# levayz/ProtoSAM

Measured on AMD Instinct MI355X. Metric: query-slices/sec (512x512) end-to-end ProtoSAM infer, higher is better.
Workload: dtype f16

## Files before the change

### include/protosam_hip.h

```cpp
#ifndef PROTOSAM_HIP_H
#define PROTOSAM_HIP_H
#include <stddef.h>
#ifdef __cplusplus
extern "C" {
#endif

int psam_gemm_f16(const void* A, const void* W, const float* bias, void* out, const float* resid, const float* gamma,
                  int M, int N, int K, int lda, int ldw, int ldo, int ldr, int resid_mod, int out_seg,
                  int out_seg_stride, int out_seg_off, int epilogue, void* stream);
int psam_gemm_f16_heads(const void* A, const void* W, const float* bias, void* out, int M, int N, int K, int lda, int ldw,
                        int hd, void* stream);
int psam_gemm_f16_ln(const void* A, const void* W, const float* bias, void* out, const float* resid, const float* gamma,
                     int M, int N, int K, int lda, int ldw, int ldo, int ldr, int resid_mod, int out_seg,
                     int out_seg_stride, int out_seg_off, int epilogue, void* out16, int ld16, float* stats,
                     const float* ln_mr, const float* ln_s, void* stream);
int psam_ln_finalize(const float* stats, int M, int D, float eps, float* mr, void* stream);


int psam_gemm_splitk_ranges(int M, int N, int K);
int psam_gemm_f16_splitk_ln(const void* A, const void* W, const float* bias, float* x, int M, int N, int K, int lda, int ldw, int ldx,
                            int ks, float* ws, const float* ln_w, const float* ln_b, float eps, void* out16, int ld16, void* stream);

int psam_gemm_set_tile(int tile);
int psam_gemm_last_tile(int* tile);
// ... 23 lines not shown
#define PSAM_ATTN_KERNEL_STAGE64 0x200
#define PSAM_ATTN_KERNEL_QT4 0x400
#define PSAM_ATTN_KERNEL_V2 0x800
int psam_attention_last_kernel(int* id);
int psam_attention_fused_relpos(int B, int N, int H, int hd, int gh, int gw);

int psam_relpos(const void* qkv, const void* Rpack, float* rel_h, float* rel_w, void* relq, int B, int N, int H, int hd,
                int gw, int K, int windowed, float scale, int head_major, void* stream);

int psam_alp_bank(const float* sup, int ld, int h, int w, int C, const float* mask, const float* bmask, int MH, int MW,
                  int pool_w, int kernel_size, float thresh, float eps, float* bank, int cap, int* meta, int* slot_bg,
                  int* slot_fg, float* mres, int force_mode, void* stream);

int psam_alp_sim(const float* qry, long long q_bstride, int ld, int B, int npix, int C, const float* bank, int cap,
                 const int* meta, float eps, float sim_scale, float* part, float* pred, int which_only, void* stream);
int psam_alp_sim_pairs(const float* qry, long long q_bstride, int ld, int npix, int C, const void* tab, int n_entries,
                       int max_groups, float eps, float sim_scale, float* part, float* pred, void* stream);

int psam_patchify_bilinear(const float* img, int B, int C, int H, int W, int S, int P, int Kpad, void* out, void* stream);
int psam_bilinear_nchw(const float* in, int planes, int IH, int IW, int OH, int OW, float* out, void* stream);
int psam_resize2d(const float* in, int planes, int IH, int IW, int OH, int OW, int mode, float* out, void* stream);
int psam_bilinear_tokens(const float* in, long long in_bstride, int ld, int B, int ih, int iw, int C, int oh, int ow,
                         float* out, void* stream);
int psam_prob_argmax(const float* logits, int B, int IH, int IW, int OH, int OW, float* prob, void* pred, int* fg_sum,
                     void* stream);
int psam_broadcast_rows(const float* row, int D, float* out, int B, long long stride, long long off, void* stream);
int psam_prob2_argmax(const float* scores, int P, int IH, int IW, int OH, int OW, void* pred, float* pfg2, int* fg_sum,
                      float* prob, void* stream);
int psam_scores_prob_argmax(const float* scores, int P, int GH, int GW, int IH, int IW, int OH, int OW, float* prob, void* pred,
                            int* fg_sum, void* stream);
int psam_minmax(const float* x, int B, long long n_per_img, void* mm, void* stream);
int psam_sam_patchify(const float* img, const void* mm, int B, int S, int P, const float* mean3, const float* std3,
                      int quantise, void* out, void* u8out, void* stream);
int psam_normalize_chw(const void* x, int in_u8, int B, long long plane, const float* mean3, const float* std3,
                       float* y, void* stream);
int psam_im2col3x3(const void* in, int B, int H, int W, int C, void* out, void* stream);
int psam_cast_f16(const float* x, void* y, long long n, void* stream);
int psam_cast_f32(const void* x, float* y, long long n, void* stream);
int psam_gelu_f32(float* x, long long n, void* stream);
int psam_split_f16(const float* x, void* hi, void* lo, long long n, int write_hi, void* stream);

int psam_ccl(const void* pred, const float* pfg, int H, int W, int cap, int* labels, int* parent, int* counters,
             int* roots, int* acc_i, void* acc_u, double* acc_d, const int* fg_sum, double* tab, void* stream);
int psam_ccl_batch(const void* pred, const float* pfg, long long pfg_stride, int B, int H, int W, int cap, int* labels, int* parent,
                   int* counters, int* roots, int* acc_i, void* acc_u, double* acc_d, const int* fg_sum, double* tab, void* stream);

int psam_small_linear(const float* x, const float* x2, const float* W, const float* b, const float* resid, float* y,
                      int G, int M, int N, int K, long long xg, long long wg, long long bg, long long yg, int ldx,
                      int ldy, int act, void* stream);
int psam_small_linear_splitk(const float* x, const float* W, const float* b, const float* resid, float* y, float* parts, int M, int N,
                             int K, int ks, int ldx, int ldy, void* stream);
int psam_small_attention(const void* q, const float* k, const float* v, void* out, int B, int Tq, int Tk, int NH, int hd,
                         int ldq, int ldk, int ldv, int ldo, int q_f16, void* stream);
#define PSAM_MAX_PROMPT_TOKENS 256
int psam_token_attention(const void* q, const float* k, const float* v, void* out, int B, int Tq, int Tk, int NH, int hd,
                         int ldq, int ldk, int ldv, int ldo, int q_f16, void* stream);
int psam_t2i_attention(const float* q, const void* K, const void* V, float* out, int B, int T, int Nk, int NH,
                       int kv_f32, void* stream);
int psam_t2i_attention_split(const float* q, const void* K, const void* V, float* out, int B, int T, int Nk, int NH,
                             int kv_f32, int S, float* part, void* stream);
int psam_gemm_f32(const float* a, const float* a2, int a2_mod, const float* w, const float* bias, const float* resid,
                  float* out, int M, int N, int K, int lda, int ldw, int ldo, void* stream);
int psam_gemm_f32_heads(const float* a, const float* a2, int a2_mod, const float* w, const float* bias, float* out, int M, int N, int K,
                        int lda, int ldw, int nk, int hd, void* stream);

int psam_gemm_f32x3(const float* a, const float* a2, int a2_mod, const void* wh, const void* wl, const float* bias, const float* resid,
// ... 67 lines not shown
```

### protosam_amd/_lib.py

```python
import ctypes
import os

import torch

_HERE = os.path.dirname(os.path.abspath(__file__))
LIB_PATH = os.environ.get("PSAM_LIB_PATH") or os.path.join(_HERE, "libprotosam_hip.so")

c_void_p, c_int, c_float, c_longlong, c_size_t = ctypes.c_void_p, ctypes.c_int, ctypes.c_float, ctypes.c_longlong, ctypes.c_size_t

SIGNATURES = {
    "psam_gemm_f16": [c_void_p, c_void_p, c_void_p, c_void_p, c_void_p, c_void_p] + [c_int] * 12 + [c_void_p],
    "psam_gemm_f16_heads": [c_void_p, c_void_p, c_void_p, c_void_p] + [c_int] * 6 + [c_void_p],
    "psam_gemm_f16_ln": [c_void_p] * 6 + [c_int] * 12 + [c_void_p, c_int, c_void_p, c_void_p, c_void_p, c_void_p],
    "psam_ln_finalize": [c_void_p, c_int, c_int, c_float, c_void_p, c_void_p],
    "psam_gemm_splitk_ranges": [c_int, c_int, c_int],
    "psam_gemm_f16_splitk_ln": [c_void_p, c_void_p, c_void_p, c_void_p] + [c_int] * 7 + [c_void_p, c_void_p, c_void_p, c_float, c_void_p, c_int,
                                c_void_p],
    "psam_gemm_set_tile": [c_int],
    "psam_gemm_last_tile": [ctypes.POINTER(c_int)],
    "psam_gemm_asm_variant": [c_int],
    "psam_gemm_set_option": [ctypes.c_char_p, c_int],
    "psam_gemm_set_workspace": [c_void_p, c_size_t],
    "psam_layernorm": [c_void_p, c_void_p, c_void_p, c_void_p, c_void_p, c_int, c_int, c_int, c_int, c_float,
                       c_int, c_int, c_void_p],
# ... 44 lines not shown
                        c_void_p, c_void_p],
    "psam_im2col": [c_void_p] + [c_int] * 10 + [c_void_p, c_void_p],
    "psam_im2col_stem": [c_void_p, c_int, c_int, c_int, c_int, c_void_p, c_void_p],
    "psam_maxpool3x3s2": [c_void_p, c_int, c_int, c_int, c_int, c_void_p, c_void_p],
    "psam_rotate_nearest": [c_void_p, c_void_p, c_void_p, c_void_p, c_void_p, c_int, c_int, c_int, c_int, c_int, c_int,
                            c_int, c_void_p],
    "psam_resize_aa": [c_void_p, c_void_p, c_void_p, c_int, c_int, c_int, c_int, c_int, c_void_p],
    "psam_image_intake": [c_void_p, c_longlong, ctypes.POINTER(c_longlong), c_void_p, c_int, c_int, c_int, c_int, c_int,
                          ctypes.POINTER(c_float), ctypes.POINTER(c_float), c_void_p, c_void_p],
    "psam_volume_stats": [c_void_p, c_int, ctypes.c_longlong, c_float, c_float, c_void_p, c_void_p],
    "psam_volume_slices": [c_void_p, c_int, c_int, c_int, c_int, c_float, c_float, c_float, c_float, c_int, c_int, c_int,
                           c_void_p, c_void_p],
    "psam_neg_points": [c_void_p, c_void_p, c_void_p, c_int, c_int, c_int, c_int, c_float, c_void_p, c_void_p],
    "psam_neg_points_batch": [c_void_p, c_void_p, c_longlong, c_void_p] + [c_int] * 6 + [c_float, c_void_p, c_void_p],
    "psam_topk_points_workspace": [c_int, c_int, c_int, ctypes.POINTER(c_longlong)],
    "psam_topk_points_batch": [c_void_p, c_void_p, c_longlong, c_void_p] + [c_int] * 7 + [c_void_p, c_void_p, c_longlong, c_void_p],
    "psam_topk_points": [c_void_p, c_void_p, c_void_p] + [c_int] * 6 + [c_void_p, c_void_p, c_longlong, c_void_p],
    "psam_mask_downscale": [c_void_p, c_void_p, c_int, c_int, c_float, c_void_p, c_void_p],
    "psam_plane_stats": [c_void_p, c_int, c_int, c_int, c_float, c_float, c_void_p, c_void_p, c_void_p],
    "psam_rle_workspace": [c_int, c_int, ctypes.POINTER(c_longlong)],
    "psam_rle_count": [c_void_p, c_int, c_int, c_int, c_void_p, c_void_p, c_void_p],
    "psam_rle_write": [c_void_p, c_int, c_int, c_int, c_void_p, c_void_p, c_void_p, c_void_p],
    "psam_rle_decode": [c_void_p, c_void_p, c_int, c_int, c_int, c_void_p, c_void_p],
    "psam_seg_counts": [c_void_p, c_int, c_int, c_longlong, c_void_p, c_int, c_int, c_longlong, c_int, c_int, c_void_p, c_int,
                        c_void_p, c_void_p],
    "psam_mask_binarize": [c_void_p, c_void_p, c_int, c_int, c_int, c_int, c_int, c_int, c_float, c_void_p, c_void_p,
                           c_void_p, c_void_p],
    "psam_normalize_chw": [c_void_p, c_int, c_int, c_longlong, ctypes.POINTER(c_float), ctypes.POINTER(c_float),
                           c_void_p, c_void_p],
    "psam_ccl": [c_void_p, c_void_p, c_int, c_int, c_int] + [c_void_p] * 9 + [c_void_p],
    "psam_ccl_batch": [c_void_p, c_void_p, c_longlong, c_int, c_int, c_int, c_int] + [c_void_p] * 9 + [c_void_p],
    "psam_sam_patchify": [c_void_p, c_void_p, c_int, c_int, c_int, ctypes.POINTER(c_float), ctypes.POINTER(c_float),
                          c_int, c_void_p, c_void_p, c_void_p],
}

_lib = None


class HipExtensionMissing(RuntimeError):
    pass


def _preload_torch_hip_runtime():
    tl = os.path.join(os.path.dirname(torch.__file__), "lib", "libamdhip64.so")
    if os.path.exists(tl):
        ctypes.CDLL(tl, mode=ctypes.RTLD_GLOBAL)


def lib():
    global _lib
    if _lib is not None:
        return _lib
    if not os.path.exists(LIB_PATH):
        raise HipExtensionMissing(
            f"{LIB_PATH} not found: build it with `make -C protosam_amd/csrc` (or __graft_entry__.build()). "
            "protosam_amd has no CPU fallback.")
    _preload_torch_hip_runtime()
    L = ctypes.CDLL(LIB_PATH)
    for name, argtypes in SIGNATURES.items():
        fn = getattr(L, name)
        fn.argtypes = argtypes
        fn.restype = c_int
    _lib = L
    return L


# ... 4 lines not shown
```

### protosam_amd/csrc/resample.hip

```cpp
#include "common.h"
#include "interp.h"

__global__ void patchify_bilinear_kernel(const float* __restrict__ img, int B, int C, int H, int W, int S, int P,
                                         int Kpad, half_t* __restrict__ out) {
  const int npw = S / P;
  const int patch = blockIdx.x, b = blockIdx.y;
  const int py = patch / npw, px = patch % npw;
  const float sh = (float)H / (float)S, sw = (float)W / (float)S;
  half_t* o = out + ((size_t)b * npw * npw + patch) * Kpad;
  const int K = C * P * P;
  const bool same = (H == S && W == S);
  for (int k = threadIdx.x; k < Kpad; k += blockDim.x) {
    float v = 0.f;
    if (k < K) {
      int c = k / (P * P), r = k % (P * P);
      int y = py * P + r / P, x = px * P + r % P;
      const float* pl = img + ((size_t)b * C + c) * H * W;
      if (same) {
        v = pl[(size_t)y * W + x];
      } else {
        Lin ly = lin_src(y, sh, H), lx = lin_src(x, sw, W);
        v = bilerp(pl, W, ly, lx);
      }
    }
// ... 158 lines not shown
}
__global__ __launch_bounds__(256) void minmax_kernel(const float* __restrict__ x, size_t n_per_img,
                                                     uint32_t* __restrict__ mm) {
  const int b = blockIdx.y;
  const float* p = x + (size_t)b * n_per_img;
  float lo = INFINITY, hi = -INFINITY;
  const size_t n4 = ((reinterpret_cast<uintptr_t>(p) & 15) == 0) ? n_per_img / 4 : 0;
  for (size_t i = (size_t)blockIdx.x * blockDim.x + threadIdx.x; i < n4; i += (size_t)gridDim.x * blockDim.x) {
    const float4 v = reinterpret_cast<const float4*>(p)[i];
    lo = fminf(fminf(lo, v.x), fminf(fminf(v.y, v.z), v.w));
    hi = fmaxf(fmaxf(hi, v.x), fmaxf(fmaxf(v.y, v.z), v.w));
  }
  for (size_t i = n4 * 4 + (size_t)blockIdx.x * blockDim.x + threadIdx.x; i < n_per_img; i += (size_t)gridDim.x * blockDim.x) {
    float v = p[i];
    lo = fminf(lo, v);
    hi = fmaxf(hi, v);
  }
  lo = wave_min(lo);
  hi = wave_max(hi);
  __shared__ float red[2][4];
  if ((threadIdx.x & 63) == 0) {
    red[0][threadIdx.x >> 6] = lo;
    red[1][threadIdx.x >> 6] = hi;
  }
  __syncthreads();
  if (threadIdx.x == 0) {
    lo = fminf(fminf(red[0][0], red[0][1]), fminf(red[0][2], red[0][3]));
    hi = fmaxf(fmaxf(red[1][0], red[1][1]), fmaxf(red[1][2], red[1][3]));
    atomicMin(&mm[2 * b], f2ord(lo));
    atomicMax(&mm[2 * b + 1], f2ord(hi));
  }
}

__global__ void sam_patchify_kernel(const float* __restrict__ img, const uint32_t* __restrict__ mm, int S, int P,
                                    float m0, float m1, float m2, float s0, float s1, float s2, int quantise,
                                    half_t* __restrict__ out, uint8_t* __restrict__ u8out) {
  const int npw = S / P;
  const int patch = blockIdx.x, b = blockIdx.y;
  const int py = patch / npw, px = patch % npw;
  const float lo = ord2f(mm[2 * b]), hi = ord2f(mm[2 * b + 1]);
  const float rng = hi - lo;
  const int K = 3 * P * P;
  half_t* o = out + ((size_t)b * npw * npw + patch) * K;
  for (int k = threadIdx.x; k < K; k += blockDim.x) {
    int c = k / (P * P), r = k % (P * P);
    int y = py * P + r / P, x = px * P + r % P;
    float v = img[(((size_t)b * 3 + c) * S + y) * S + x];
    float q = (v - lo) / rng;
    if (quantise) {
      q = q * 255.0f;
      q = (float)(int)q;
      if (u8out) u8out[(((size_t)b * 3 + c) * S + y) * S + x] = (uint8_t)q;
    }
    const float mean = c == 0 ? m0 : (c == 1 ? m1 : m2);
    const float sd = c == 0 ? s0 : (c == 1 ? s1 : s2);
    o[k] = (half_t)((q - mean) / sd);
  }
}

extern "C" int psam_minmax(const float* x, int B, long long n_per_img, void* mm, void* stream) {
  if (B <= 0 || n_per_img <= 0) return PSAM_ERR_ARG;
  hipStream_t s = (hipStream_t)stream;
  hipLaunchKernelGGL(minmax_init_kernel, dim3((B + 63) / 64), dim3(64), 0, s, (uint32_t*)mm, B);
  int nb = (int)((n_per_img + 256 * 16 - 1) / (256 * 16));
  if (nb > 128) nb = 128;
  hipLaunchKernelGGL(minmax_kernel, dim3(nb, B), dim3(256), 0, s, x, (size_t)n_per_img, (uint32_t*)mm);
  return psam_launch_status();
}

extern "C" int psam_sam_patchify(const float* img, const void* mm, int B, int S, int P, const float* mean3,
                                 const float* std3, int quantise, void* out, void* u8out, void* stream) {
  if (B <= 0 || S <= 0 || P <= 0 || S % P || !mean3 || !std3) return PSAM_ERR_ARG;
  const int np = (S / P) * (S / P);
  hipLaunchKernelGGL(sam_patchify_kernel, dim3(np, B), dim3(256), 0, (hipStream_t)stream, img, (const uint32_t*)mm, S,
                     P, mean3[0], mean3[1], mean3[2], std3[0], std3[1], std3[2], quantise, (half_t*)out,
                     (uint8_t*)u8out);
  return psam_launch_status();
}

__global__ void im2col3x3_kernel(const half_t* __restrict__ in, int H, int W, int C, half_t* __restrict__ out) {
  const int pix = blockIdx.x, b = blockIdx.y;
  const int y = pix / W, x = pix % W;
  const int cv = C / 8;
  uint4* o = reinterpret_cast<uint4*>(out + ((size_t)b * H * W + pix) * 9 * C);
  for (int i = threadIdx.x; i < 9 * cv; i += blockDim.x) {
    int tap = i / cv, c = i % cv;
    int yy = y + tap / 3 - 1, xx = x + tap % 3 - 1;
    uint4 v = make_uint4(0, 0, 0, 0);
    if (yy >= 0 && yy < H && xx >= 0 && xx < W)
      v = reinterpret_cast<const uint4*>(in + ((size_t)b * H * W + (size_t)yy * W + xx) * C)[c];
    o[i] = v;
  }
}
extern "C" int psam_im2col3x3(const void* in, int B, int H, int W, int C, void* out, void* stream) {
  if (B <= 0 || H <= 0 || W <= 0 || C <= 0 || (C % 8) != 0) return PSAM_ERR_ARG;
  hipLaunchKernelGGL(im2col3x3_kernel, dim3(H * W, B), dim3(256), 0, (hipStream_t)stream, (const half_t*)in, H, W, C,
                     (half_t*)out);
  return psam_launch_status();
}

__global__ void cast_f16_kernel(const float* __restrict__ x, half_t* __restrict__ y, size_t n8) {
  size_t i = (size_t)blockIdx.x * blockDim.x + threadIdx.x;
  if (i >= n8) return;
  const float4 a = reinterpret_cast<const float4*>(x)[2 * i], b = reinterpret_cast<const float4*>(x)[2 * i + 1];
  half8_t h = {(half_t)a.x, (half_t)a.y, (half_t)a.z, (half_t)a.w, (half_t)b.x, (half_t)b.y, (half_t)b.z, (half_t)b.w};
  reinterpret_cast<half8_t*>(y)[i] = h;
}
extern "C" int psam_cast_f16(const float* x, void* y, long long n, void* stream) {
// ... 303 lines not shown
```

### protosam_amd/ops.py

```python
import torch

from . import _lib

EPI_F16, EPI_GELU_F16, EPI_F32, EPI_RELU_F16 = 0, 1, 2, 3


_raw_stream = getattr(torch._C, "_cuda_getCurrentRawStream", None)
_raw_device = getattr(torch._C, "_cuda_getDevice", None)


def _stream():
    if _raw_stream is not None and _raw_device is not None:
        return _raw_stream(_raw_device())
    return torch.cuda.current_stream().cuda_stream


class KernelTimer:

    def __init__(self):
        self.records = []
        self.tags = {}

    def start(self):
        e = torch.cuda.Event(enable_timing=True)
# ... 630 lines not shown
    st = _lib.lib().psam_prob2_argmax(_ptr(scores), P, scores.shape[2], scores.shape[3], OH, OW, _ptr(pred), _ptr(pfg2),
                                      _ptr(fg_sum), _ptr(prob), _stream())
    _tstop(h, P * (2 * scores.shape[2] * scores.shape[3] * 4 + OH * OW * (5 + (8 if prob is not None else 0))))
    _lib.check(st, "psam_prob2_argmax")
    return pred, pfg2


def scores_prob_argmax(scores, IH, IW, OH, OW, prob=None, pred=None, fg_sum=None):
    _req(scores, torch.float32, "scores")
    assert scores.is_contiguous() and scores.dim() == 4 and scores.shape[1] == 2
    P, dev = scores.shape[0], scores.device
    if prob is None:
        prob = torch.empty((P, 2, OH, OW), dtype=torch.float32, device=dev)
    if pred is None:
        pred = torch.empty((P, OH, OW), dtype=torch.uint8, device=dev)
    _req(prob, torch.float32, "prob")
    assert prob.is_contiguous() and prob.numel() >= P * 2 * OH * OW
    assert pred.dtype == torch.uint8 and pred.is_cuda and pred.is_contiguous() and pred.numel() >= P * OH * OW
    assert fg_sum is None or (fg_sum.dtype == torch.int32 and fg_sum.is_cuda and fg_sum.is_contiguous() and fg_sum.numel() >= P)
    h = _tstart("scores_prob_argmax")
    st = _lib.lib().psam_scores_prob_argmax(_ptr(scores), P, scores.shape[2], scores.shape[3], IH, IW, OH, OW, _ptr(prob),
                                            _ptr(pred), _ptr(fg_sum), _stream())
    _tstop(h, P * (2 * scores.shape[2] * scores.shape[3] * 4 + OH * OW * 9))
    _lib.check(st, "psam_scores_prob_argmax")
    return prob, pred


def broadcast_rows(row, out, B, stride, off):
    _req(row, torch.float32, "row"); _req(out, torch.float32, "out")
    st = _lib.lib().psam_broadcast_rows(_ptr(row), row.numel(), _ptr(out), B, stride, off, _stream())
    _lib.check(st, "psam_broadcast_rows")


def minmax(x, B, mm=None):
    _req(x, torch.float32, "x")
    assert x.is_contiguous()
    if mm is None:
        mm = torch.empty(2 * B, dtype=torch.int32, device=x.device)
    st = _lib.lib().psam_minmax(_ptr(x), B, x.numel() // B, _ptr(mm), _stream())
    _lib.check(st, "psam_minmax")
    return mm


def sam_patchify(img, mm, S, P, mean3, std3, quantise=True, out=None, u8out=None):
    import ctypes
    _req(img, torch.float32, "img")
    assert img.is_contiguous() and img.shape[-1] == S and img.shape[-2] == S
    B = img.shape[0]
    if out is None:
        out = torch.empty((B * (S // P) ** 2, 3 * P * P), dtype=torch.float16, device=img.device)
    m = (ctypes.c_float * 3)(*[float(v) for v in mean3])
    s = (ctypes.c_float * 3)(*[float(v) for v in std3])
    st = _lib.lib().psam_sam_patchify(_ptr(img), _ptr(mm), B, S, P, m, s, 1 if quantise else 0, _ptr(out), _ptr(u8out),
                                     _stream())
    _lib.check(st, "psam_sam_patchify")
    return out


def im2col3x3(x, B, H, W, C, out=None):
    _req(x, torch.float16, "x")
    assert x.is_contiguous()
    if out is None:
        out = torch.empty((B * H * W, 9 * C), dtype=torch.float16, device=x.device)
    st = _lib.lib().psam_im2col3x3(_ptr(x), B, H, W, C, _ptr(out), _stream())
    _lib.check(st, "psam_im2col3x3")
    return out


def cast_f16(x, out=None):
    _req(x, torch.float32, "x")
    assert x.is_contiguous()
    if out is None:
        out = torch.empty(x.shape, dtype=torch.float16, device=x.device)
    _req_aligned(x, 16, "x"); _req_aligned(out, 16, "out")
    st = _lib.lib().psam_cast_f16(_ptr(x), _ptr(out), x.numel(), _stream())
    _lib.check(st, "psam_cast_f16")
    return out


def cast_f32(x, out=None):
    _req(x, torch.float16, "x")
    assert x.is_contiguous()
    if out is None:
        out = torch.empty(x.shape, dtype=torch.float32, device=x.device)
    _req(out, torch.float32, "out")
# ... 753 lines not shown
```

### protosam_amd/protomedsam.py

```python
import numpy as np
import torch
import torch.nn as nn

from . import ops
from .protosam import CCL_SLOTS, DECODER_CHUNK, MAX_COMPONENTS, ModelWrapper, ProtoSAM, class_support_scores
from .segment_anything import sam_model_registry


class ProtoMedSAM(nn.Module):
    _coarse_logits = ProtoSAM._coarse_logits
    _coarse_only_batch = ProtoSAM._coarse_only_batch
    _ccl_large = ProtoSAM._ccl_large

    def __init__(self, image_size, coarse_segmentation_model: ModelWrapper,
                 sam_pretrained_path="pretrained_model/medsam_vit_b.pth", debug=False, use_cca=False,
                 coarse_pred_only=False):
        super().__init__()
        if isinstance(image_size, int):
            image_size = (image_size, image_size)
        self.image_size = image_size
        self.coarse_segmentation_model = coarse_segmentation_model
        self.get_sam(sam_pretrained_path)
        self.coarse_pred_only = coarse_pred_only
        self.debug = debug
# ... 72 lines not shown
    @torch.no_grad()
    def segment_all(self, query_image, query_label):
        H, W = query_image.shape[-2:]
        sam = self.medsam
        S = sam.image_encoder.img_size
        if (H, W) != (S, S):
            raise ValueError(f"segment_all: the image encoder takes {S} x {S} images, got {(H, W)}")
        bbox = np.array([[0, 0, W, H]])
        g = sam.image_encoder.grid
        emb = self._medsam_features(query_image, self._batch_bufs(query_image.device, 1, 1)).view(1, g, g, -1).permute(0, 3, 1, 2)
        medsam_seg, conf = self.medsam_inference(emb, bbox, H, W, query_label)
        medsam_seg = torch.tensor(medsam_seg, device=query_image.device)
        return medsam_seg.view(H, W), [conf]

    @torch.no_grad()
    def forward(self, query_image, coarse_model_input, degrees_rotate=0):
        return self.forward_batch(query_image, coarse_model_input, degrees_rotate)[0]

    @torch.no_grad()
    def forward_classes(self, query_image, support_image, support_masks, val_wsize=2):
        return self.forward_classes_batch(query_image, support_image, support_masks, val_wsize)[0]

    def _batch_bufs(self, dev, P, B):
        S = self.medsam.image_encoder.img_size
        bb = self.__dict__.setdefault("_bbufs", {})
        if bb.get("P", 0) < P:
            bb.update(P=P, pred=None, pfg2=None)
            bb.update(pred=torch.empty((P, S, S), dtype=torch.uint8, device=dev),
                      pfg2=torch.empty((P, S, S), dtype=torch.float32, device=dev),
                      fg=torch.zeros(P, dtype=torch.int32, device=dev), fg_host=torch.zeros(P, dtype=torch.int32).pin_memory(),
                      tabs_host=torch.empty((P, ops.CC_HDR + ops.CC_STRIDE * MAX_COMPONENTS), dtype=torch.float64).pin_memory(),
                      fg_event=torch.cuda.Event(), event=torch.cuda.Event())
        if bb.get("B", 0) < B:
            bb.update(B=B, q1024=None)
            bb.update(q1024=torch.empty((B, 3, S, S), dtype=torch.float32, device=dev),
                      mm=torch.empty(2 * B, dtype=torch.int32, device=dev),
                      patches=torch.empty((B * 4096, 768), dtype=torch.float16, device=dev))
        slots = min(P, CCL_SLOTS)
        if getattr(self, "_ccl_chunk", None) is None or self._ccl_chunk.slots < slots:
            self._ccl_chunk = None
            self._ccl_chunk = ops.CclWorkspace(S, S, MAX_COMPONENTS, dev, slots=slots)
        return bb

    def _coarse_to_components(self, scores, P, bb):
        S = self.medsam.image_encoder.img_size
        pred, pfg2, fg = bb["pred"][:P], bb["pfg2"][:P], bb["fg"][:P]
        fg.zero_()
        ops.prob2_argmax(scores, S, S, pred=pred, pfg2=pfg2, fg_sum=fg)
        bb["fg_host"][:P].copy_(fg, non_blocking=True)
        bb["fg_event"].record()
        cw = self._ccl_chunk
        for c0 in range(0, P, cw.slots):
            c1 = min(c0 + cw.slots, P)
            ops.ccl_planes(pred[c0:c1], pfg2[c0:c1], cw, fg_sum=fg[c0:c1])
            bb["tabs_host"][c0:c1].copy_(cw.tabs[:c1 - c0], non_blocking=True)
        bb["event"].record()

    def _medsam_features(self, imgs, bb):
        sam = self.medsam
        S = sam.image_encoder.img_size
        n = imgs.shape[0]
        q = imgs.float().contiguous()
        if tuple(q.shape[-2:]) != (S, S):
            q = ops.bilinear_nchw(q, S, S, out=bb["q1024"][:n])
        mm, patches = bb["mm"][:2 * n], bb["patches"][:n * 4096]
        ops.minmax(q, n, mm=mm)
        ops.sam_patchify(q, mm, S, sam.image_encoder.patch_size, (0.0, 0.0, 0.0), (1.0, 1.0, 1.0), False, out=patches)
        return sam.image_encoder.encode_patches(patches, n)

    def _decode_boxes(self, feat_tok, boxes, img_idx):
        sam = self.medsam
        S = sam.image_encoder.img_size
        dev = feat_tok.device
        n = len(boxes)
        coords = torch.from_numpy(np.stack(boxes).reshape(-1, 2, 2).astype(np.float32)).to(dev)
        labels = torch.from_numpy(np.tile(np.array([[2, 3]], dtype=np.int32), (n, 1))).to(dev)
        iop = torch.tensor(img_idx, dtype=torch.int32).to(dev)
        pe = sam.prompt_encoder._packed()
        dpk = sam.mask_decoder._packed()
        tokens = ops.prompt_tokens(coords, labels, pe["G"], pe["type_emb"], dpk["out_tok"], n, 2, float(S))
        masks = torch.empty((n, 4, 256, 256), dtype=torch.float32, device=dev)
        iou = torch.empty((n, 4), dtype=torch.float32, device=dev)
        for c0 in range(0, n, DECODER_CHUNK):
            c1 = min(c0 + DECODER_CHUNK, n)
            sam.mask_decoder.predict_masks_tokens(feat_tok, pe["pe_tok"], tokens[c0:c1].contiguous(), pe["no_mask"],
                                                  img_of_prompt=iop[c0:c1].contiguous(), masks_out=masks[c0:c1],
                                                  iou_out=iou[c0:c1])
        return masks, iou

    def _segment(self, query_images, scores, C, relabel, out=None):
        B, H = query_images.shape[0], query_images.shape[-2]
        P = C * B
        dev = query_images.device
        S = self.medsam.image_encoder.img_size
        bb = self._batch_bufs(dev, P, B)
        self._coarse_to_components(scores, P, bb)
        bb["fg_event"].synchronize()
        fgh = bb["fg_host"][:P].view(C, B)
        keep = [b for b in range(B) if int(fgh[:, b].max()) > 0]
# ... 82 lines not shown
```

### protosam_amd/protosam.py

```python
import os
from abc import ABC, abstractmethod
from functools import partial

import numpy as np
import torch
import torch.nn as nn

from . import ops
from .grid_proto_fewshot import FewShotSeg
from .rotate import reverse_tensor, rotate_tensor_no_crop
from .sam_wrapper import SamWrapper
from .segment_anything import SamPredictor, sam_model_registry
from .segment_anything.utils.transforms import ResizeLongestSide

CONF_MODE = "conf"
CENTROID_MODE = "centroid"
BOTH_MODE = "both"
POINT_MODES = (CONF_MODE, CENTROID_MODE, BOTH_MODE)

TYPE_ALPNET = "alpnet"
TYPE_SAM = "sam"

MAX_COMPONENTS = 256
MAX_COMPONENTS_LARGE = 4096
# ... 438 lines not shown
                if self.use_neg_points:
                    ring = ops.decode_point_key(int(neg_keys[1 + first + k]), 1024)
                    if ring is None and glob is None:
                        raise TypeError("'NoneType' object is not iterable")
                    for pt in (ring, glob):
                        if pt is not None:
                            c.append([float(pt[0]), float(pt[1])])
                            lab.append(0)
                if not self.use_bbox:
                    c.append([0.0, 0.0])
                    lab.append(-1)
            if self.use_bbox:
                c += [[r[3], r[4]], [r[5], r[6]]]
                lab += [2, 3]
            coords.append(c)
            labels.append(lab)
        return coords, labels, rows

    def _batch_bufs(self, dev, P, B):
        S = self.sam.image_encoder.img_size
        bb = self.__dict__.setdefault("_bbufs", {})
        if bb.get("P", 0) < P:
            bb.update(P=P, prob=None, pred=None, lab256=None)
            bb.update(prob=torch.empty((P, 2, S, S), dtype=torch.float32, device=dev),
                      pred=torch.empty((P, S, S), dtype=torch.uint8, device=dev),
                      fg_sum=torch.zeros(P, dtype=torch.int32, device=dev), fg_host=torch.zeros(P, dtype=torch.int32).pin_memory(),
                      tabs_host=torch.empty((P, ops.CC_HDR + ops.CC_STRIDE * MAX_COMPONENTS), dtype=torch.float64).pin_memory(),
                      neg_keys=torch.empty((P, MAX_NEG_COMPONENTS + 1), dtype=torch.int64, device=dev),
                      neg_keys_host=torch.empty((P, MAX_NEG_COMPONENTS + 1), dtype=torch.int64).pin_memory(),
                      topk_keys=None, topk_keys_host=None,
                      lab256=torch.empty((P, S // 4, S // 4), dtype=torch.int32, device=dev) if self._mask_only else None,
                      fg_event=torch.cuda.Event(), event=torch.cuda.Event(), sam_done=torch.cuda.Event())
        if bb.get("B", 0) < B:
            bb.update(B=B, q1024=None, patches=None)
            bb.update(q1024=torch.empty((B, 3, S, S), dtype=torch.float32, device=dev),
                      mm=torch.empty(2 * B, dtype=torch.int32, device=dev),
                      patches=torch.empty((B * 4096, 768), dtype=torch.float16, device=dev))
        shape = (bb["P"], 1 if self.use_cca else MAX_TOPK_COMPONENTS, self.num_points_for_sam)
        if self.topk_points == "device" and self._wants_topk() and (bb["topk_keys"] is None or bb["topk_keys"].shape != shape):
            bb.update(topk_keys=torch.empty(shape, dtype=torch.int64, device=dev),
                      topk_keys_host=torch.empty(shape, dtype=torch.int64).pin_memory())
        slots = min(P, CCL_SLOTS)
        if bb.get("ccl") is None or bb["ccl"].slots < slots:
            bb["ccl"] = None
            bb["ccl"] = ops.CclWorkspace(S, S, MAX_COMPONENTS, dev, slots=slots)
        return bb

    def _ccl_large(self, pred, pfg, fg_sum):
        H, W = pred.shape
        big = self.__dict__.setdefault("_ccl_big", {})
        if (H, W) not in big:
            big[(H, W)] = ops.CclWorkspace(H, W, MAX_COMPONENTS_LARGE, pred.device, slots=1)
        ws = ops.ccl(pred, pfg, big[(H, W)], fg_sum=fg_sum, slot=0)
        tab = ws.tabs[0].cpu().numpy()
        if int(tab[0]) > int(tab[1]):
            raise RuntimeError(f"{int(tab[0])} connected components in one coarse mask exceed the table capacity "
                               f"{MAX_COMPONENTS_LARGE} (csrc/ccl.hip)")
        return ws, tab

    def _side_stream(self, dev):
        if getattr(self, "_side", None) is None:
            self._side = torch.cuda.Stream(device=dev)
        return self._side

    def _sam_features(self, query_images, bufs, B, S):
        sam = self.sam
        q = query_images.float().contiguous()
        if tuple(q.shape[-2:]) != (S, S):
            q = ops.bilinear_nchw(q, S, S, out=bufs["q1024"][:B])
        mm, patches = bufs["mm"][:2 * B], bufs["patches"][:B * 4096]
        ops.minmax(q, B, mm=mm)
        enc = sam.image_encoder
        if getattr(enc, "split_fp16", False) or getattr(enc, "gemm_x3", False):
            ops.sam_patchify(q, mm, S, enc.patch_size, (0.0, 0.0, 0.0), (1.0, 1.0, 1.0), True, out=patches)
            return enc.encode_patches(patches, B, raw_norm=(tuple(sam._mean_host), tuple(sam._std_host)))
        ops.sam_patchify(q, mm, S, enc.patch_size, sam._mean_host, sam._std_host, True, out=patches)
        return enc.encode_patches(patches, B)

    def forward(self, query_image, coarse_model_input, degrees_rotate=0):
        if self.training:
            raise NotImplementedError("training-mode outputs (logits) are outside the inference hot path")
        return self.forward_batch(query_image, coarse_model_input, degrees_rotate)[0]

    def _coarse_logits(self, query_images, coarse_model_input, degrees_rotate=0):
        if isinstance(coarse_model_input, (list, tuple)):
            if degrees_rotate != 0:
                raise NotImplementedError("rotation TTA with a mixed-support batch")
            alp = getattr(self.coarse_segmentation_model, "model", None)
            if not hasattr(alp, "forward_groups"):
                raise TypeError("a list of (input, count) pairs needs a coarse model with forward_groups (ALPNetWrapper(FewShotSeg))")
            return alp.forward_groups(query_images, [(i.supp_imgs, i.fore_mask, i.back_mask, i.isval, i.val_wsize, n)
                                                     for i, n in coarse_model_input])
        if degrees_rotate == 0:
            coarse_model_input.set_query_images(query_images)
            return self.coarse_segmentation_model(coarse_model_input)
        rotated, (rot_h, rot_w) = rotate_tensor_no_crop(query_images, degrees_rotate)
        coarse_model_input.set_query_images(rotated)
        logits_rot = self.coarse_segmentation_model(coarse_model_input)
        return reverse_tensor(logits_rot, rot_h, rot_w, -degrees_rotate)

    @torch.no_grad()
    def forward_batch(self, query_images, coarse_model_input, degrees_rotate=0):
        B, H = query_images.shape[0], query_images.shape[-2]
        dev = query_images.device
        if self.coarse_pred_only:
            return self._coarse_only_batch(self._coarse_logits(query_images, coarse_model_input, degrees_rotate), H)
        bb = self._batch_bufs(dev, B, B)
        S = self.sam.image_encoder.img_size
        main = torch.cuda.current_stream(dev)
        mode = self.overlap_streams
        if isinstance(mode, str):
            mode = True if mode == "1" else False if mode == "0" else (self._dense_run >= 4 and STAGE_TIMER is None and not ops.TIMERS and ops.GEMM_TIMER is None)
        feat_tok = None
        if mode:
            side = self._side_stream(dev)
            side.wait_stream(main)
            with torch.cuda.stream(side):
                feat_tok = self._sam_features(query_images, bb, B, S)
                bb["sam_done"].record(side)
        _mark("start")
        output_logits = self._coarse_logits(query_images, coarse_model_input, degrees_rotate)
        _mark("coarse: DINOv2 + ALP")
        out, res, tabs, st = self._segment(query_images, 1, partial(ops.prob_argmax, output_logits.float().contiguous(), S, S),
                                           feat_tok=feat_tok)
        self._dense_run = self._dense_run + 1 if all(int(tab[0]) > 0 for tab in tabs) else 0
        masks = out.view(B, H, H).float()
        results, stats = [], []
        for b, tab in enumerate(tabs):
            stats.append(dict(n_components=int(tab[0]), fg_pixels=int(tab[2]), n_prompts=st["spans"].get((b, 0), (0, 0))[1]))
            if (b, 0) not in st["prompt"]:
                results.append((bb["prob"][b].argmax(dim=0), [0]))
                continue
            results.append((masks[b], res[b][0][1]))
            if not self._mask_only:
                stats[b].update(table=st["tables"][(b, 0)], prompts=st["prompts"][(b, 0)])
        self.last_stats = stats[0] if B == 1 else dict(per_slice=stats)
        if st["low_res"] is not None:
            self.last_stats.update({k: st[k] for k in ("low_res", "iou", "sel", "best") if k in st},
                                   spans=[(b, first, cnt) for (b, _), (first, cnt) in st["spans"].items()])
        return results

    def _segment(self, query_images, C, coarse, out=None, feat_tok=None):
        B, H = query_images.shape[0], query_images.shape[-2]
        P = C * B
        dev = query_images.device
        sam = self.sam
        S = sam.image_encoder.img_size
        bb = self._batch_bufs(dev, P, B)
        prob, pred, fg = bb["prob"][:P], bb["pred"][:P], bb["fg_sum"][:P]
        fg.zero_()
        coarse(prob=prob, pred=pred, fg_sum=fg)
        bb["fg_host"][:P].copy_(fg, non_blocking=True)
        bb["fg_event"].record()
        cw, pending = bb["ccl"], feat_tok is not None
        topk_dev = self._wants_topk() and self.topk_points == "device"
        need_labels = self.use_neg_points or (self._wants_topk() and not topk_dev)
        tabs_h, keys_h = bb["tabs_host"][:P], bb["neg_keys_host"][:P]
        tk_h = bb["topk_keys_host"][:P] if topk_dev else None
        sets, keep = {}, None
# ... 35 lines not shown
        for p in range(P):
            tab, big = tabs_h[p].numpy(), None
            if int(tab[0]) > int(tab[1]):
                big, tab = self._ccl_large(pred[p], prob[p, 1], fg[p:p + 1])
                if self._mask_only:
                    bb["lab256"][p].copy_(big.labels.view(S, S)[::4, ::4])
            tabs.append(tab)
            if int(tab[1]) > 0 and p not in sets:
                if topk_dev and big is None and not self.use_cca and int(tab[1]) > MAX_TOPK_COMPONENTS:
                    big = self._ccl_large(pred[p], prob[p, 1], fg[p:p + 1])[0]
                sets[p] = self._plane_prompts(tab, prob[p], None, big, plane=p,
                                              topk_keys=tk_h[p].numpy() if topk_dev and big is None else None)
        feat_row = [-1] * B
        for i, b in enumerate(keep):
            feat_row[b] = i
        prompts = {(p % B, p // B): s[:2] for p, s in sets.items()}
        plan = plan_class_prompts(B, C, prompts, feat_row)
        if pending:
            main = torch.cuda.current_stream(dev)
            main.wait_event(bb["sam_done"])
            feat_tok.record_stream(main)
        masks = iou = best = low = None
        sel, sel_u = (0 if self.use_cca else 1), 0
        if plan["labels"]:
            if self._mask_only:
                masks, iou = self._decode_mask_sets(feat_tok, bb["lab256"], plan["plane_idx"], plan["labels"], plan["img_idx"])
                best = iou[:, 1:].argmax(dim=1)
                low = masks[torch.arange(len(plan["labels"]), device=dev), best + 1].unsqueeze(1).contiguous()
                scores = iou[:, 1:].max(dim=1).values
            else:
                masks, iou = self._decode_point_sets(feat_tok, plan["coords"], plan["labels"], plan["img_idx"])
                low, sel_u, scores = masks, sel, iou[:, sel]
            _mark("prompt encoder + mask decoder")
            scores_h = scores.cpu().numpy()
        if out is None:
            out = torch.empty((B, C, H, H), dtype=torch.uint8, device=dev)
        assert out.shape == (B, C, H, H) and out.dtype == torch.uint8 and out.is_contiguous()
        segs = torch.from_numpy(plan["segs"]).to(dev)
        ops.mask_union_seg(low, sel_u, segs, P, S, H, sam.variant_id(), sam.mask_threshold, out=out.view(P, H, H))
        _mark("post-processing (upsample, threshold, union)")
        results = [[(out[b, c], [0]) for c in range(C)] for b in range(B)]
        for (b, c), (first, cnt) in plan["spans"].items():
            results[b][c] = (out[b, c], [np.float32(v) for v in scores_h[first:first + cnt]])
        stats = dict(n_slices=B, n_classes=C, prompt=plan["prompt"], spans=plan["spans"], n_prompted=len(plan["prompt"]),
                     n_encoded=len(keep), n_components=[[int(tabs[c * B + b][0]) for c in range(C)] for b in range(B)],
                     prompts=prompts, tables={(p % B, p // B): s[2] for p, s in sets.items()}, low_res=masks, iou=iou, sel=sel)
        if best is not None:
            stats.update(best=best)
        return out, results, tabs, stats

    def _plane_prompts(self, tab, prob, neg_keys, ws=None, slot=0, plane=None, topk_keys=None):
        S = self.sam.image_encoder.img_size
        n_found, n = int(tab[0]), int(tab[1])
        ids = [int(tab[3]) + 1] if self.use_cca else list(range(1, n + 1))
        if self._mask_only:
            return None, ids, None
        if self.use_neg_points and (n > MAX_NEG_COMPONENTS or n_found > MAX_COMPONENTS):
            neg_keys = ops.neg_points(ws, prob[0], ws.tabs[slot], n, labels=ws.labels_b[slot]).cpu().numpy()
        topk = None
        if self._wants_topk() and self.topk_points == "device":
            if topk_keys is None or (not self.use_cca and n > MAX_TOPK_COMPONENTS):
                topk_keys = ops.topk_points(ws, prob[1], ws.tabs[slot], self.num_points_for_sam, n, only_best=self.use_cca,
                                            labels=ws.labels_b[slot]).cpu().numpy()
            topk = self._topk_from_keys(topk_keys, tab, ids, plane)
        elif self._wants_topk():
            topk = self._topk_points(prob[1], ws.labels_b[slot], S, ids, self.num_points_for_sam)
        return self._prompts_from_table(tab, neg_keys, topk)

    @torch.no_grad()
    def forward_classes_batch(self, query_images, support_image=None, support_masks=None, val_wsize=2, out=None, degrees_rotate=0,
                              supports=None):
        if self.training:
            raise NotImplementedError("training-mode outputs (logits) are outside the inference hot path")
# ... 133 lines not shown
```

### protosam_amd/runner.py

```python
import math

import numpy as np
import torch
import torch.distributed as dist

from .grid_proto_fewshot import FewShotSeg
from .metrics import class_rows
from .protosam import ALPNetWrapper, InputFactory, ProtoSAM, TYPE_ALPNET
from .synth import synth_state_dict

ALP_CFG = {"which_model": "dinov2_b14", "cls_name": "grid_proto", "proto_grid_size": 8, "lora": 0, "align": False,
           "debug": False}


def build_protosam(device, sam_type="vit_h", image_size=512, seed=1234, dino_depth=None, sam_depth=None,
                   cache_support=True, heavy_tail=False, **protosam_kw):
    cfg = dict(ALP_CFG)
    if dino_depth is not None:
        cfg["encoder_depth"] = dino_depth
    alp = FewShotSeg(image_size, None, cfg, cache_support=cache_support)
    alp_sd = synth_state_dict(alp, seed)
    alp.load_state_dict(alp_sd)
    alp = alp.to(device).eval()
    spec = ("random-heavy" if heavy_tail else "random") + f":{sam_type}:{seed}" + (f":{sam_depth}" if sam_depth is not None else "")
# ... 22 lines not shown
def shard_slices(n_slices, rank, world):
    return list(range(rank, n_slices, world))


def _batch_dst(out, buf, i, j):
    return out[i:j] if out is not None else buf[:j - i]


@torch.no_grad()
def run_slices(model, vol, sup_imgs, sup_masks, zs, device, out=None, batch=1, mix_parts=True):
    if out is None:
        out = torch.zeros((len(zs), vol.shape[-1], vol.shape[-1]), dtype=torch.uint8, device=device)
    return out, _slices_loop(model, vol, sup_imgs, sup_masks, zs, device, out, None, batch, mix_parts, None)


def _slices_loop(model, vol, sup_imgs, sup_masks, zs, device, out, buf, batch, mix_parts, sink):
    n, S = vol.shape[0], vol.shape[-1]
    stats = [0] * len(zs)
    inputs = {}

    def part_input(part, q):
        if part not in inputs:
            inputs[part] = InputFactory.create_input(TYPE_ALPNET, q, support_images=[sup_imgs[part]],
                                                     support_labels=[sup_masks[part]], isval=True, val_wsize=2)
        return inputs[part]
    i = 0
    while i < len(zs):
        part = part_assign(zs[i], n)
        j = i
        while j < len(zs) and j - i < batch and (mix_parts and batch > 1 or part_assign(zs[j], n) == part):
            j += 1
        idx = torch.tensor(zs[i:j], device=device)
        q = vol[idx][:, None].expand(j - i, 3, S, S).contiguous()
        if batch == 1:
            res = [model(q, part_input(part, q), degrees_rotate=0)]
            st = [model.last_stats]
        else:
            runs = []
            for z in zs[i:j]:
                pz = part_assign(z, n)
                if runs and runs[-1][0] == pz:
                    runs[-1][1] += 1
                else:
                    runs.append([pz, 1])
            cin = part_input(part, q) if len(runs) == 1 else [(part_input(pz, q), cnt) for pz, cnt in runs]
            res = model.forward_batch(q, cin)
            st = model.last_stats.get("per_slice", [model.last_stats])
        dst = _batch_dst(out, buf, i, j)
        for k, (pred, scores) in enumerate(res):
            if pred.shape[-1] == S:
                dst[k].copy_(pred)
            else:
                dst[k].zero_()
            stats[i + k] = st[k].get("n_prompts", 0) if k < len(st) else 0
        if sink is not None:
            sink(i, j, dst)
        i = j
    return stats


@torch.no_grad()
def run_slices_classes(model, vol, sup_imgs, sup_masks_per_part, zs, device, batch=16, out=None):
    if out is None:
        out = torch.zeros((len(zs), len(sup_masks_per_part[0]), vol.shape[-1], vol.shape[-1]), dtype=torch.uint8, device=device)
    return out, _slices_classes_loop(model, vol, sup_imgs, sup_masks_per_part, zs, device, batch, out, None, None)


def _collect_classes(model, res, dst, stats, i):
    for k, per_class in enumerate(res):
        for c, (mask, _) in enumerate(per_class):
            if mask.data_ptr() != dst[k, c].data_ptr():
                dst[k, c].copy_(mask)
    for (k, _) in model.last_stats.get("prompt", {}):
        stats[i + k] += 1


def _slices_classes_loop(model, vol, sup_imgs, sup_masks_per_part, zs, device, batch, out, buf, sink):
    n, S = vol.shape[0], vol.shape[-1]
    stats = [0] * len(zs)
    i = 0
    while i < len(zs):
        part = part_assign(zs[i], n)
        j = i
        while j < len(zs) and j - i < batch and part_assign(zs[j], n) == part:
            j += 1
        idx = torch.tensor(zs[i:j], device=device)
# ... 208 lines not shown
```

Before: 168.3.

## Fuse bilinear resize into minmax and patchify; write batch masks in place

Removes the separate bilinear upsample of the query images to SAM resolution, which wrote a full-size float intermediate. The min/max and patchify kernels now interpolate on the fly. forward_batch also gains an out buffer so the runner's uint8 destination is filled directly, avoiding the per-slice float mask plus copy. The host sync that pulls scores back is moved after post-processing and skipped when there are no prompts. The cost is recomputing bilinear taps in both minmax and patchify.

```diff
diff --git a/include/protosam_hip.h b/include/protosam_hip.h
--- a/include/protosam_hip.h
+++ b/include/protosam_hip.h
@@ -79,6 +79,9 @@
 int psam_minmax(const float* x, int B, long long n_per_img, void* mm, void* stream);
 int psam_sam_patchify(const float* img, const void* mm, int B, int S, int P, const float* mean3, const float* std3,
                       int quantise, void* out, void* u8out, void* stream);
+int psam_minmax_resized(const float* x, int B, int C, int IH, int IW, int OH, int OW, void* mm, void* stream);
+int psam_sam_patchify_resized(const float* img, const void* mm, int B, int IH, int IW, int S, int P, const float* mean3,
+                              const float* std3, int quantise, void* out, void* u8out, void* stream);
 int psam_normalize_chw(const void* x, int in_u8, int B, long long plane, const float* mean3, const float* std3,
                        float* y, void* stream);
 int psam_im2col3x3(const void* in, int B, int H, int W, int C, void* out, void* stream);
diff --git a/protosam_amd/_lib.py b/protosam_amd/_lib.py
--- a/protosam_amd/_lib.py
+++ b/protosam_amd/_lib.py
@@ -100,6 +100,9 @@
     "psam_ccl_batch": [c_void_p, c_void_p, c_longlong, c_int, c_int, c_int, c_int] + [c_void_p] * 9 + [c_void_p],
     "psam_sam_patchify": [c_void_p, c_void_p, c_int, c_int, c_int, ctypes.POINTER(c_float), ctypes.POINTER(c_float),
                           c_int, c_void_p, c_void_p, c_void_p],
+    "psam_minmax_resized": [c_void_p] + [c_int] * 6 + [c_void_p, c_void_p],
+    "psam_sam_patchify_resized": [c_void_p, c_void_p] + [c_int] * 5 + [ctypes.POINTER(c_float), ctypes.POINTER(c_float),
+                                                                     c_int, c_void_p, c_void_p, c_void_p],
 }
 
 _lib = None
diff --git a/protosam_amd/csrc/resample.hip b/protosam_amd/csrc/resample.hip
--- a/protosam_amd/csrc/resample.hip
+++ b/protosam_amd/csrc/resample.hip
@@ -214,8 +214,41 @@
   }
 }
 
-__global__ void sam_patchify_kernel(const float* __restrict__ img, const uint32_t* __restrict__ mm, int S, int P,
-                                    float m0, float m1, float m2, float s0, float s1, float s2, int quantise,
+__global__ __launch_bounds__(256) void minmax_resized_kernel(const float* __restrict__ x, int C, int IH, int IW, int OH,
+                                                             int OW, uint32_t* __restrict__ mm) {
+  const int b = blockIdx.z;
+  const int ox = blockIdx.x * blockDim.x + threadIdx.x;
+  const float sh = (float)IH / (float)OH, sw = (float)IW / (float)OW;
+  float lo = INFINITY, hi = -INFINITY;
+  if (ox < OW) {
+    const Lin lx = lin_src(ox, sw, IW);
+    for (int oy = blockIdx.y; oy < OH; oy += gridDim.y) {
+      const Lin ly = lin_src(oy, sh, IH);
+      for (int c = 0; c < C; ++c) {
+        const float v = bilerp(x + ((size_t)b * C + c) * IH * IW, IW, ly, lx);
+        lo = fminf(lo, v);
+        hi = fmaxf(hi, v);
+      }
+    }
+  }
+  lo = wave_min(lo);
+  hi = wave_max(hi);
+  __shared__ float red[2][4];
+  if ((threadIdx.x & 63) == 0) {
+    red[0][threadIdx.x >> 6] = lo;
+    red[1][threadIdx.x >> 6] = hi;
+  }
+  __syncthreads();
+  if (threadIdx.x == 0) {
+    lo = fminf(fminf(red[0][0], red[0][1]), fminf(red[0][2], red[0][3]));
+    hi = fmaxf(fmaxf(red[1][0], red[1][1]), fmaxf(red[1][2], red[1][3]));
+    atomicMin(&mm[2 * b], f2ord(lo));
+    atomicMax(&mm[2 * b + 1], f2ord(hi));
+  }
+}
+
+__global__ void sam_patchify_kernel(const float* __restrict__ img, const uint32_t* __restrict__ mm, int IH, int IW, int S,
+                                    int P, float m0, float m1, float m2, float s0, float s1, float s2, int quantise,
                                     half_t* __restrict__ out, uint8_t* __restrict__ u8out) {
   const int npw = S / P;
   const int patch = blockIdx.x, b = blockIdx.y;
@@ -223,11 +256,19 @@
   const float lo = ord2f(mm[2 * b]), hi = ord2f(mm[2 * b + 1]);
   const float rng = hi - lo;
   const int K = 3 * P * P;
+  const bool same = (IH == S && IW == S);
+  const float sh = (float)IH / (float)S, sw = (float)IW / (float)S;
   half_t* o = out + ((size_t)b * npw * npw + patch) * K;
   for (int k = threadIdx.x; k < K; k += blockDim.x) {
     int c = k / (P * P), r = k % (P * P);
     int y = py * P + r / P, x = px * P + r % P;
-    float v = img[(((size_t)b * 3 + c) * S + y) * S + x];
+    float v;
+    if (same) {
+      v = img[(((size_t)b * 3 + c) * S + y) * S + x];
+    } else {
+      Lin ly = lin_src(y, sh, IH), lx = lin_src(x, sw, IW);
+      v = bilerp(img + ((size_t)b * 3 + c) * IH * IW, IW, ly, lx);
+    }
     float q = (v - lo) / rng;
     if (quantise) {
       q = q * 255.0f;
@@ -250,12 +291,31 @@
   return psam_launch_status();
 }
 
+extern "C" int psam_minmax_resized(const float* x, int B, int C, int IH, int IW, int OH, int OW, void* mm, void* stream) {
+  if (B <= 0 || C <= 0 || IH <= 0 || IW <= 0 || OH <= 0 || OW <= 0) return PSAM_ERR_ARG;
+  hipStream_t s = (hipStream_t)stream;
+  hipLaunchKernelGGL(minmax_init_kernel, dim3((B + 63) / 64), dim3(64), 0, s, (uint32_t*)mm, B);
+  const int ny = OH < 32 ? OH : 32;
+  hipLaunchKernelGGL(minmax_resized_kernel, dim3((OW + 255) / 256, ny, B), dim3(256), 0, s, x, C, IH, IW, OH, OW,
+                     (uint32_t*)mm);
+  return psam_launch_status();
+}
+
+extern "C" int psam_sam_patchify_resized(const float* img, const void* mm, int B, int IH, int IW, int S, int P,
+                                         const float* mean3, const float* std3, int quantise, void* out, void* u8out,
+                                         void* stream);
 extern "C" int psam_sam_patchify(const float* img, const void* mm, int B, int S, int P, const float* mean3,
                                  const float* std3, int quantise, void* out, void* u8out, void* stream) {
-  if (B <= 0 || S <= 0 || P <= 0 || S % P || !mean3 || !std3) return PSAM_ERR_ARG;
+  return psam_sam_patchify_resized(img, mm, B, S, S, S, P, mean3, std3, quantise, out, u8out, stream);
+}
+
+extern "C" int psam_sam_patchify_resized(const float* img, const void* mm, int B, int IH, int IW, int S, int P,
+                                         const float* mean3, const float* std3, int quantise, void* out, void* u8out,
+                                         void* stream) {
+  if (B <= 0 || IH <= 0 || IW <= 0 || S <= 0 || P <= 0 || S % P || !mean3 || !std3) return PSAM_ERR_ARG;
   const int np = (S / P) * (S / P);
-  hipLaunchKernelGGL(sam_patchify_kernel, dim3(np, B), dim3(256), 0, (hipStream_t)stream, img, (const uint32_t*)mm, S,
-                     P, mean3[0], mean3[1], mean3[2], std3[0], std3[1], std3[2], quantise, (half_t*)out,
+  hipLaunchKernelGGL(sam_patchify_kernel, dim3(np, B), dim3(256), 0, (hipStream_t)stream, img, (const uint32_t*)mm, IH,
+                     IW, S, P, mean3[0], mean3[1], mean3[2], std3[0], std3[1], std3[2], quantise, (half_t*)out,
                      (uint8_t*)u8out);
   return psam_launch_status();
 }
diff --git a/protosam_amd/ops.py b/protosam_amd/ops.py
--- a/protosam_amd/ops.py
+++ b/protosam_amd/ops.py
@@ -686,11 +686,16 @@
     _lib.check(st, "psam_broadcast_rows")
 
 
-def minmax(x, B, mm=None):
+def minmax(x, B, mm=None, size=None):
     _req(x, torch.float32, "x")
     assert x.is_contiguous()
     if mm is None:
         mm = torch.empty(2 * B, dtype=torch.int32, device=x.device)
+    if size is not None and tuple(size) != tuple(x.shape[-2:]):
+        assert x.dim() == 4 and x.shape[0] == B
+        st = _lib.lib().psam_minmax_resized(_ptr(x), B, x.shape[1], x.shape[2], x.shape[3], size[0], size[1], _ptr(mm), _stream())
+        _lib.check(st, "psam_minmax_resized")
+        return mm
     st = _lib.lib().psam_minmax(_ptr(x), B, x.numel() // B, _ptr(mm), _stream())
     _lib.check(st, "psam_minmax")
     return mm
@@ -699,12 +704,17 @@
 def sam_patchify(img, mm, S, P, mean3, std3, quantise=True, out=None, u8out=None):
     import ctypes
     _req(img, torch.float32, "img")
-    assert img.is_contiguous() and img.shape[-1] == S and img.shape[-2] == S
-    B = img.shape[0]
+    assert img.is_contiguous() and img.dim() == 4 and img.shape[1] == 3
+    B, IH, IW = img.shape[0], img.shape[-2], img.shape[-1]
     if out is None:
         out = torch.empty((B * (S // P) ** 2, 3 * P * P), dtype=torch.float16, device=img.device)
     m = (ctypes.c_float * 3)(*[float(v) for v in mean3])
     s = (ctypes.c_float * 3)(*[float(v) for v in std3])
+    if (IH, IW) != (S, S):
+        st = _lib.lib().psam_sam_patchify_resized(_ptr(img), _ptr(mm), B, IH, IW, S, P, m, s, 1 if quantise else 0, _ptr(out),
+                                                 _ptr(u8out), _stream())
+        _lib.check(st, "psam_sam_patchify_resized")
+        return out
     st = _lib.lib().psam_sam_patchify(_ptr(img), _ptr(mm), B, S, P, m, s, 1 if quantise else 0, _ptr(out), _ptr(u8out),
                                      _stream())
     _lib.check(st, "psam_sam_patchify")
diff --git a/protosam_amd/protomedsam.py b/protosam_amd/protomedsam.py
--- a/protosam_amd/protomedsam.py
+++ b/protosam_amd/protomedsam.py
@@ -128,9 +128,8 @@
                       tabs_host=torch.empty((P, ops.CC_HDR + ops.CC_STRIDE * MAX_COMPONENTS), dtype=torch.float64).pin_memory(),
                       fg_event=torch.cuda.Event(), event=torch.cuda.Event())
         if bb.get("B", 0) < B:
-            bb.update(B=B, q1024=None)
-            bb.update(q1024=torch.empty((B, 3, S, S), dtype=torch.float32, device=dev),
-                      mm=torch.empty(2 * B, dtype=torch.int32, device=dev),
+            bb.update(B=B, patches=None)
+            bb.update(mm=torch.empty(2 * B, dtype=torch.int32, device=dev),
                       patches=torch.empty((B * 4096, 768), dtype=torch.float16, device=dev))
         slots = min(P, CCL_SLOTS)
         if getattr(self, "_ccl_chunk", None) is None or self._ccl_chunk.slots < slots:
@@ -157,10 +156,8 @@
         S = sam.image_encoder.img_size
         n = imgs.shape[0]
         q = imgs.float().contiguous()
-        if tuple(q.shape[-2:]) != (S, S):
-            q = ops.bilinear_nchw(q, S, S, out=bb["q1024"][:n])
         mm, patches = bb["mm"][:2 * n], bb["patches"][:n * 4096]
-        ops.minmax(q, n, mm=mm)
+        ops.minmax(q, n, mm=mm, size=(S, S))
         ops.sam_patchify(q, mm, S, sam.image_encoder.patch_size, (0.0, 0.0, 0.0), (1.0, 1.0, 1.0), False, out=patches)
         return sam.image_encoder.encode_patches(patches, n)
 
diff --git a/protosam_amd/protosam.py b/protosam_amd/protosam.py
--- a/protosam_amd/protosam.py
+++ b/protosam_amd/protosam.py
@@ -494,9 +494,8 @@
                       lab256=torch.empty((P, S // 4, S // 4), dtype=torch.int32, device=dev) if self._mask_only else None,
                       fg_event=torch.cuda.Event(), event=torch.cuda.Event(), sam_done=torch.cuda.Event())
         if bb.get("B", 0) < B:
-            bb.update(B=B, q1024=None, patches=None)
-            bb.update(q1024=torch.empty((B, 3, S, S), dtype=torch.float32, device=dev),
-                      mm=torch.empty(2 * B, dtype=torch.int32, device=dev),
+            bb.update(B=B, patches=None)
+            bb.update(mm=torch.empty(2 * B, dtype=torch.int32, device=dev),
                       patches=torch.empty((B * 4096, 768), dtype=torch.float16, device=dev))
         shape = (bb["P"], 1 if self.use_cca else MAX_TOPK_COMPONENTS, self.num_points_for_sam)
         if self.topk_points == "device" and self._wants_topk() and (bb["topk_keys"] is None or bb["topk_keys"].shape != shape):
@@ -528,10 +527,8 @@
     def _sam_features(self, query_images, bufs, B, S):
         sam = self.sam
         q = query_images.float().contiguous()
-        if tuple(q.shape[-2:]) != (S, S):
-            q = ops.bilinear_nchw(q, S, S, out=bufs["q1024"][:B])
         mm, patches = bufs["mm"][:2 * B], bufs["patches"][:B * 4096]
-        ops.minmax(q, B, mm=mm)
+        ops.minmax(q, B, mm=mm, size=(S, S))
         enc = sam.image_encoder
         if getattr(enc, "split_fp16", False) or getattr(enc, "gemm_x3", False):
             ops.sam_patchify(q, mm, S, enc.patch_size, (0.0, 0.0, 0.0), (1.0, 1.0, 1.0), True, out=patches)
@@ -562,11 +559,17 @@
         return reverse_tensor(logits_rot, rot_h, rot_w, -degrees_rotate)
 
     @torch.no_grad()
-    def forward_batch(self, query_images, coarse_model_input, degrees_rotate=0):
+    def forward_batch(self, query_images, coarse_model_input, degrees_rotate=0, out=None):
         B, H = query_images.shape[0], query_images.shape[-2]
         dev = query_images.device
+        if out is not None and not (out.dtype == torch.uint8 and out.is_contiguous() and tuple(out.shape) == (B, H, H)):
+            raise ValueError(f"out: a contiguous uint8 [{B}, {H}, {H}] tensor")
         if self.coarse_pred_only:
-            return self._coarse_only_batch(self._coarse_logits(query_images, coarse_model_input, degrees_rotate), H)
+            res = self._coarse_only_batch(self._coarse_logits(query_images, coarse_model_input, degrees_rotate), H)
+            if out is not None:
+                for b, (pred, _) in enumerate(res):
+                    out[b].copy_(pred)
+            return res
         bb = self._batch_bufs(dev, B, B)
         S = self.sam.image_encoder.img_size
         main = torch.cuda.current_stream(dev)
@@ -583,10 +586,10 @@
         _mark("start")
         output_logits = self._coarse_logits(query_images, coarse_model_input, degrees_rotate)
         _mark("coarse: DINOv2 + ALP")
-        out, res, tabs, st = self._segment(query_images, 1, partial(ops.prob_argmax, output_logits.float().contiguous(), S, S),
-                                           feat_tok=feat_tok)
+        u8, res, tabs, st = self._segment(query_images, 1, partial(ops.prob_argmax, output_logits.float().contiguous(), S, S),
+                                          feat_tok=feat_tok, out=None if out is None else out.view(B, 1, H, H))
         self._dense_run = self._dense_run + 1 if all(int(tab[0]) > 0 for tab in tabs) else 0
-        masks = out.view(B, H, H).float()
+        masks = u8.view(B, H, H).float() if out is None else out
         results, stats = [], []
         for b, tab in enumerate(tabs):
             stats.append(dict(n_components=int(tab[0]), fg_pixels=int(tab[2]), n_prompts=st["spans"].get((b, 0), (0, 0))[1]))
@@ -688,13 +691,14 @@
                 masks, iou = self._decode_point_sets(feat_tok, plan["coords"], plan["labels"], plan["img_idx"])
                 low, sel_u, scores = masks, sel, iou[:, sel]
             _mark("prompt encoder + mask decoder")
-            scores_h = scores.cpu().numpy()
         if out is None:
             out = torch.empty((B, C, H, H), dtype=torch.uint8, device=dev)
         assert out.shape == (B, C, H, H) and out.dtype == torch.uint8 and out.is_contiguous()
         segs = torch.from_numpy(plan["segs"]).to(dev)
         ops.mask_union_seg(low, sel_u, segs, P, S, H, sam.variant_id(), sam.mask_threshold, out=out.view(P, H, H))
         _mark("post-processing (upsample, threshold, union)")
+        if plan["labels"]:
+            scores_h = scores.cpu().numpy()
         results = [[(out[b, c], [0]) for c in range(C)] for b in range(B)]
         for (b, c), (first, cnt) in plan["spans"].items():
             results[b][c] = (out[b, c], [np.float32(v) for v in scores_h[first:first + cnt]])
diff --git a/protosam_amd/runner.py b/protosam_amd/runner.py
--- a/protosam_amd/runner.py
+++ b/protosam_amd/runner.py
@@ -78,6 +78,8 @@
             j += 1
         idx = torch.tensor(zs[i:j], device=device)
         q = vol[idx][:, None].expand(j - i, 3, S, S).contiguous()
+        dst = _batch_dst(out, buf, i, j)
+        direct = batch > 1 and isinstance(model, ProtoSAM)
         if batch == 1:
             res = [model(q, part_input(part, q), degrees_rotate=0)]
             st = [model.last_stats]
@@ -90,14 +92,14 @@
                 else:
                     runs.append([pz, 1])
             cin = part_input(part, q) if len(runs) == 1 else [(part_input(pz, q), cnt) for pz, cnt in runs]
-            res = model.forward_batch(q, cin)
+            res = model.forward_batch(q, cin, out=dst) if direct else model.forward_batch(q, cin)
             st = model.last_stats.get("per_slice", [model.last_stats])
-        dst = _batch_dst(out, buf, i, j)
         for k, (pred, scores) in enumerate(res):
-            if pred.shape[-1] == S:
-                dst[k].copy_(pred)
-            else:
-                dst[k].zero_()
+            if not direct:
+                if pred.shape[-1] == S:
+                    dst[k].copy_(pred)
+                else:
+                    dst[k].zero_()
             stats[i + k] = st[k].get("n_prompts", 0) if k < len(st) else 0
         if sink is not None:
             sink(i, j, dst)
```

Measured after the change: 168.3. About the same (-0.0%).
